# AdmiralenOla/Scoary

Measured on AMD Instinct MI355X. Metric: gene x permutation Fisher tests/sec, higher is better.
Workload: dtype u32 bit-words (bit-sliced adders / AND + popcount), f64 for Fisher p; 1 GPU; cfg3: 50000 genes x 2000 isolates x 10 traits, --permute 10000 per GPU; counts + Fisher + label permutations + exceedance counts; gene_kind=config, gene_order=config, gene_partition=every rank its own genes (weak scaling), genes_per_gpu=50000, genes_total=50000, isolates=2000, traits=10, permutations=10000, parallelism=gene-shard x1, hip_graph=False, hip_graph_auto=False, label_tiles=generated on every rank, exchange=none (single GPU)

## Files before the change

### scoary_amd/csrc/scoary_mfma.hip

```cpp
#include "scoary_common.hpp"

const double kMfmaNsPerGene = 58.0;
const double kListNsPerEntry = 0.18;
const double kMfmaBlockStartStages = 6.0;
const double kMfmaTraitSwitchStages = 2.0;

namespace {

typedef int v8i __attribute__((ext_vector_type(8)));
typedef float v4f __attribute__((ext_vector_type(4)));

constexpr int kBlockGenes = 256;
constexpr int kBlockWaves = 8;
constexpr int kHalfBytes = kStageBytes / 2;
constexpr int kKSteps128 = kKSteps / 2;
constexpr int kKStepBytes = kStageBytes / kKSteps128;
constexpr int kRingSlots = 4;
constexpr int kAhead = kRingSlots - 2;
constexpr int kRingBytes = kRingSlots * kHalfBytes;
constexpr int kDmaPerHalf = kHalfBytes / kBlockWaves / kFragBytes;
constexpr int kThrBytes = 32 * 8;
constexpr int kMfmaLds = kRingBytes + kBlockWaves * kThrBytes;
static_assert(kRingSlots >= 4 && kMfmaLds <= 160 * 1024 && (kAhead - 1) * kDmaPerHalf < 64,
              "a half stage is issued at least two ticks ahead, within the LDS of a CU and the vmcnt field");

__global__ __launch_bounds__(256) void k_mfma_panels(const uint32_t* __restrict__ tiled, int64_t Gp, int G, int N,
                                                     const int32_t* __restrict__ order,
                                                     const uint8_t* __restrict__ flipped, int64_t total,
                                                     v4i* __restrict__ panels) {
  const int64_t idx = (int64_t)blockIdx.x * 256 + threadIdx.x;
  if (idx >= total) return;
  const int lane = (int)(idx & 63);
  const int64_t f = idx >> 6;
  const int k = (int)(f & 31), i = (int)((f >> 5) & 1);
  const int64_t slot = (f >> 6) * 64 + i * 32 + (lane & 31);
  const int w = 2 * k + (lane >> 5);
  uint32_t bits = 0u;
  if (slot < G && 32 * w < N) {
    const int g = order[slot];
    bits = tiled[((int64_t)(w >> 2) * Gp + g) * 4 + (w & 3)];
    if (flipped[g]) bits = ~bits;
    if (32 * w + 32 > N) bits &= (1u << (N - 32 * w)) - 1u;
  }
  panels[idx] = fp4_of_bits32(bits);
}

__global__ __launch_bounds__(256) void k_mfma_bfrag(const uint32_t* __restrict__ tiles, int N, int ntiles,
                                                    int64_t tile_dwords, int S, v4i* __restrict__ bfrag) {
  const int s = blockIdx.x, t = blockIdx.y;
  const int wave = __builtin_amdgcn_readfirstlane(threadIdx.x >> 6);
  const uint32_t* tile = tiles + ((int64_t)t * ntiles + (s >> 3)) * tile_dwords + 2 * (s & 7);
#pragma unroll
  for (int j = 0; j < 2; ++j)
    mfma_bfrag_emit(bfrag, S, t, s, j, wave, 4, [&](int row) { return row < N ? tile[(int64_t)row * 16 + j] : 0u; });
}

__device__ __forceinline__ void mfma_dma16(uint32_t lds, uint32_t lane_off, const unsigned char* src) {
  uint32_t m0_saved;
  asm volatile("s_mov_b32 %0, m0\n\ts_mov_b32 m0, %1\n\ts_nop 0\n\t"
               "global_load_lds_dwordx4 %2, %3\n\ts_mov_b32 m0, %0"
               : "=&s"(m0_saved)
               : "s"(lds), "v"(lane_off), "s"(src)
               : "memory");
}

__device__ __forceinline__ void mfma_dma4(uint32_t lds, uint32_t lane_off, const unsigned char* src) {
  uint32_t m0_saved;
  asm volatile("s_mov_b32 %0, m0\n\ts_mov_b32 m0, %1\n\ts_nop 0\n\t"
               "global_load_lds_dword %2, %3\n\ts_mov_b32 m0, %0"
               : "=&s"(m0_saved)
               : "s"(lds), "v"(lane_off), "s"(src)
               : "memory");
}

__device__ __forceinline__ int xcd_item(int orig, int n) {
  const int q = n >> 3, r = n & 7, x = orig & 7;
  return (x < r ? x * (q + 1) : r * (q + 1) + (x - r) * q) + (orig >> 3);
}

__global__ __launch_bounds__(kBlockWaves * 64) __attribute__((amdgpu_waves_per_eu(2, 2)))
void k_permute_mfma(const v4i* __restrict__ panels, const unsigned char* __restrict__ bfrag,
                    const uint2* __restrict__ lcrit, int G, int64_t P, int S, int64_t Q, int L, int nblk_genes,
                    int ntiles, int64_t gs, uint16_t* __restrict__ partial) {
  extern __shared__ __attribute__((aligned(16))) unsigned char lds[];
  const int item = xcd_item(blockIdx.x, gridDim.x);
  const int gb = item % nblk_genes, rng = item / nblk_genes;
  const int64_t q0 = (int64_t)rng * L;
  const int ns = (int)min((int64_t)L, Q - q0);
  int t = (int)(q0 / S), s = (int)(q0 % S);
  int jt = rng - (int)((int64_t)t * S / L);
  const int tid = threadIdx.x, lane = tid & 63, quad = lane >> 4, l15 = lane & 15;
  const int wave = __builtin_amdgcn_readfirstlane(tid >> 6);
  const bool late = wave >= kBlockWaves / 2;
  const int wslot0 = gb * kBlockGenes + wave * 32;
  const int rows_mine = min(32, G - wslot0) - 4 * quad;
  v4f negc[2];
  float hw[8];
  const uint32_t lds0 = (uint32_t)(uintptr_t)(const __attribute__((address_space(3))) unsigned char*)lds;
  const uint32_t lane_off = (uint32_t)lane * 16u;
  const int thr_slot0 = min(wslot0, G - 1);
  const uint32_t thr_lds = kRingBytes + (uint32_t)wave * kThrBytes;
  auto fetch_thresholds = [&](int tt) {
    uint32_t l = lane_off;
    asm volatile("" : "+v"(l));
    l >>= 4;
    const uint32_t off = (uint32_t)min((int)(l >> 1), G - 1 - thr_slot0) * 8u + (l & 1u) * 4u;
    mfma_dma4(lds0 + thr_lds, off, reinterpret_cast<const unsigned char*>(lcrit + ((int64_t)tt * G + thr_slot0)));
  };
  auto take_thresholds = [&]() {
    int q4 = 4 * quad, mine = rows_mine;
    asm volatile("" : "+v"(q4), "+v"(mine));
    const uint2* thr = reinterpret_cast<const uint2*>(lds + thr_lds) + q4;
#pragma unroll
    for (int r = 0; r < 8; ++r) {
      const int row = 16 * (r >> 2) + (r & 3);
      const uint2 cr = thr[row];
      negc[r >> 2][r & 3] = -0.5f * (float)((int)cr.x + (int)cr.y - 1);
      hw[r] = row < mine ? 0.5f * (float)((int)cr.y - 1 - (int)cr.x) : 1e30f;
    }
    asm volatile("" : "+v"(negc[0]), "+v"(negc[1]));
#pragma unroll
    for (int r = 0; r < 8; ++r) asm volatile("" : "+v"(hw[r]));
  };
  v4i a[2][kKSteps128];
  {
    fetch_thresholds(t);
    const v4i* ap = panels + ((int64_t)gb * kBlockWaves + wave) * (kKSteps * 64) + (quad >> 1) * 64 + (quad & 1) * 32 + l15;
#pragma unroll
    for (int k = 0; k < kKSteps128; ++k)
#pragma unroll
      for (int i = 0; i < 2; ++i) a[i][k] = ap[k * 128 + i * 16];
#pragma unroll
    for (int k = 0; k < kKSteps128; ++k) asm volatile("" : "+v"(a[0][k]), "+v"(a[1][k]));
    asm volatile("s_waitcnt vmcnt(0)" ::: "memory");
    take_thresholds();
  }

  const unsigned char* bsrc = bfrag + q0 * kStageBytes + wave * (kHalfBytes / kBlockWaves);
  const int nh = 2 * ns;
  auto issue_half = [&](int n) {
    const unsigned char* src = bsrc + (int64_t)min(n, nh - 1) * kHalfBytes;
    const uint32_t dst = lds0 + (uint32_t)(n % kRingSlots) * kHalfBytes + (uint32_t)wave * (kHalfBytes / kBlockWaves);
#pragma unroll
    for (int p = 0; p < kDmaPerHalf; ++p) mfma_dma16(dst + p * kFragBytes, lane_off, src + p * kFragBytes);
  };
#pragma unroll
  for (int n = 0; n < kAhead; ++n) issue_half(n);
  int tick = 0;
  auto next_tick = [&]() {
    asm volatile("s_waitcnt vmcnt(%0)" ::"n"((kAhead - 1) * kDmaPerHalf) : "memory");
    __builtin_amdgcn_s_barrier();
    issue_half(tick + kAhead);
    ++tick;
  };

  uint32_t ex[8];
#pragma unroll
  for (int r = 0; r < 8; ++r) ex[r] = 0u;
  const int ragged = (int)(P - (int64_t)(S - 1) * 64);

  v4f acc[2][4];
  auto region_test = [&](int nvalid) {
    if (nvalid < 64) {
#pragma unroll
      for (int j = 0; j < 4; ++j) {
        const bool v = 16 * j + l15 < nvalid;
#pragma unroll
        for (int r = 0; r < 8; ++r) acc[r >> 2][j][r & 3] = v ? acc[r >> 2][j][r & 3] : __builtin_nanf("");
      }
    }
#pragma unroll
    for (int r = 0; r < 8; ++r)
#pragma unroll
      for (int j = 0; j < 4; ++j) ex[r] += (uint32_t)(__builtin_fabsf(acc[r >> 2][j][r & 3]) > hw[r]);
  };
  const int jt0 = jt;
  auto end_segment = [&](int tt) {
    uint16_t* out = partial + ((int64_t)tt * ntiles + jt) * gs + wslot0;
    int rl = l15, q4 = 4 * quad, mine = rows_mine;
    asm volatile("" : "+v"(rl), "+v"(q4), "+v"(mine));
    uint32_t count = 0u;
#pragma unroll
    for (int r = 0; r < 8; ++r) {
      uint32_t v = ex[r];
#pragma unroll
      for (int off = 8; off > 0; off >>= 1) v += __shfl_xor(v, off);
      ex[r] = 0u;
      count = rl == r ? v : count;
    }
    const int row = 16 * (rl >> 2) + (rl & 3);
    if (rl < 8 && row < mine) out[q4 + row] = (uint16_t)count;
    jt = 0;
  };
  if (late) next_tick();
  int rslot = 0;
  for (int st = 0; st < ns; ++st) {
#pragma unroll
    for (int h = 0; h < 2; ++h) {
      next_tick();
      const unsigned char* bbuf = lds + rslot * kHalfBytes + ((quad >> 1) * 128 + (quad & 1) * 32 + l15) * 16;
      rslot = rslot == kRingSlots - 1 ? 0 : rslot + 1;
      constexpr int kBLead = 3, kFrags = 4 * (kKSteps128 / 2);
      v4i bq[kBLead + 1];
      auto read_b = [&](int f) {
        bq[f % (kBLead + 1)] =
            *reinterpret_cast<const v4i*>(bbuf + (f >> 2) * kKStepBytes + ((f >> 1) & 1) * kFragBytes + (f & 1) * 256);
      };
#pragma unroll
      for (int f = 0; f < kBLead; ++f) read_b(f);
      if (h == 0) {
        __builtin_amdgcn_sched_barrier(0);
        if (st > 0) {
          const bool entered = s == 0;
          region_test(entered ? ragged : 64);
          if (entered) {
            end_segment(t - 1);
            take_thresholds();
          }
        }
        if (s == S - 1 && st + 1 < ns) fetch_thresholds(t + 1);
        __builtin_amdgcn_sched_barrier(0);
      }
#pragma unroll
      for (int f = 0; f < kFrags; ++f) {
        const int k = h * (kKSteps128 / 2) + (f >> 2), j = f & 3;
        if (f + kBLead < kFrags) read_b(f + kBLead);
        __builtin_amdgcn_sched_barrier(0);
        const v4i x = bq[f % (kBLead + 1)];
        const v8i bb = v8i{x.x, x.y, x.z, x.w, 0, 0, 0, 0};
#pragma unroll
        for (int i = 0; i < 2; ++i)
          acc[i][j] = __builtin_amdgcn_mfma_scale_f32_16x16x128_f8f6f4(
              v8i{a[i][k].x, a[i][k].y, a[i][k].z, a[i][k].w, 0, 0, 0, 0}, bb, k == 0 ? negc[i] : acc[i][j], 4, 4, 0, 0,
              0, 0);
        __builtin_amdgcn_sched_barrier(0);
      }
    }
    if (++s == S) s = 0, ++t;
  }
  if (!late) next_tick();
  const bool trait_done = s == 0;
  region_test(trait_done ? ragged : 64);
  asm volatile("s_waitcnt vmcnt(0)" ::: "memory");
  end_segment(trait_done ? t - 1 : t);

  {
    int rl = l15, q4 = 4 * quad, mine = rows_mine;
    asm volatile("" : "+v"(rl), "+v"(q4), "+v"(mine));
    const int row = 16 * (rl >> 2) + (rl & 3);
    const bool stores = rl < 8 && row < mine;
    const int t0 = (int)(q0 / S);
    for (int tt = t0; tt < t; ++tt) {
      uint16_t* out = partial + (int64_t)tt * ntiles * gs + wslot0 + q4 + row;
      for (int tile = (tt == t0 ? jt0 : 0) + 1; tile < ntiles; ++tile)
        if (stores) out[(int64_t)tile * gs] = 0;
    }
  }
}

}

struct MfmaRange {
  int64_t L, ranges, switches;
};
static std::vector<MfmaRange> mfma_ranges(int64_t T, int64_t P, int64_t ntiles) {
  std::vector<MfmaRange> out;
  const int64_t S = (P + 63) / 64, Q = T * S;
  for (int64_t L = std::min<int64_t>(Q, 1023); L >= 1; --L) {
    const int64_t ranges = (Q + L - 1) / L;
    if ((Q + ranges - 1) / ranges != L) continue;
    bool ok = true;
    for (int64_t t = 0; t < std::min(T, L) && ok; ++t) ok = ((t + 1) * S - 1) / L - t * S / L + 1 <= ntiles;
    if (!ok) continue;
    MfmaRange c{L, ranges, 0};
    for (int64_t r = 0; r < std::min(ranges, S); ++r)
      c.switches = std::max(c.switches, (std::min(Q, (r + 1) * L) - 1) / S - r * L / S);
    out.push_back(c);
  }
  return out;
}

static MfmaGeom mfma_pick(const std::vector<MfmaRange>& cands, int num_cu, int64_t gene_blocks, int64_t S,
                          int64_t T) {
  MfmaGeom g{};
  g.stages = S;
  g.Q = T * S;
  g.gene_blocks = gene_blocks;
  for (const MfmaRange& c : cands) {
    const int64_t blocks = gene_blocks * c.ranges;
    const double cost = (double)((blocks + num_cu - 1) / num_cu) *
                        ((double)c.L + kMfmaBlockStartStages + (double)c.switches * kMfmaTraitSwitchStages);
    if (g.L == 0 || cost < g.cost) g.cost = cost, g.ranges = c.ranges, g.L = c.L, g.blocks = blocks;
  }
  return g;
}

MfmaGeom scoary_mfma_geom(int num_cu, int64_t k_split, int64_t T, int64_t P, int64_t ntiles) {
  return mfma_pick(mfma_ranges(T, P, ntiles), num_cu, (k_split + kBlockGenes - 1) / kBlockGenes, (P + 63) / 64, T);
}

int scoary_mfma_launch(scoary_handle h, hipStream_t s, const uint32_t* d_tiles, const void* d_panels, void* d_bfrag,
                       const uint32_t* d_lcrit, uint16_t* d_partial, int64_t k_split, int64_t G, int64_t T,
                       int64_t N, int64_t P, int64_t ntiles, int64_t gs, bool bfrag_ready) {
  const MfmaGeom g = scoary_mfma_geom(h->num_cu, k_split, T, P, ntiles);
  if (g.blocks > 0x7fffffffLL || g.stages > 0x7fffffffLL / 64)
    return fail(h, SCOARY_ERR_SIZE, "scoary_permute_hybrid: grid too large");
  if (!h->mfma_lds_optin) {
    HIP_TRY(h, hipFuncSetAttribute(reinterpret_cast<const void*>(&k_permute_mfma),
                                   hipFuncAttributeMaxDynamicSharedMemorySize, 160 * 1024));
    h->mfma_lds_optin = 1;
  }
  if (!bfrag_ready) {
    KernelTimer kt(h, s, "k_mfma_bfrag");
    hipLaunchKernelGGL(k_mfma_bfrag, dim3((unsigned)g.stages, (unsigned)T), dim3(256), 0, s, d_tiles, (int)N,
                       (int)ntiles, list_tile_dwords(N, 16), (int)g.stages, static_cast<v4i*>(d_bfrag));
  }
  {
    KernelTimer kt(h, s, "k_permute_mfma");
    hipLaunchKernelGGL(k_permute_mfma, dim3((unsigned)g.blocks), dim3(kBlockWaves * 64), kMfmaLds, s,
                       static_cast<const v4i*>(d_panels), static_cast<const unsigned char*>(d_bfrag),
                       reinterpret_cast<const uint2*>(d_lcrit), (int)G, P, (int)g.stages, g.Q, (int)g.L,
                       (int)g.gene_blocks, (int)ntiles, gs, d_partial);
  }
  HIP_TRY(h, hipGetLastError());
  return SCOARY_OK;
}

extern "C" {

int64_t scoary_mfma_max_isolates(void) { return kKSteps * 64; }
int64_t scoary_mfma_panels_bytes(int64_t G, int64_t N) {
  if (G < 1 || N < 1 || N > kKSteps * 64) return 0;
  return round_up(G, kBlockGenes) * (2 * kKSteps * 16);
}
int64_t scoary_mfma_bfrag_bytes(int64_t N, int64_t P, int64_t T) {
  if (N < 1 || N > kKSteps * 64 || P < 1 || T < 1) return 0;
  return T * ((P + 63) / 64) * kStageBytes;
}
int64_t scoary_mfma_breakeven_entries(void) { return (int64_t)std::ceil(kMfmaNsPerGene / kListNsPerEntry); }

int scoary_mfma_panels_build(scoary_handle h, const uint32_t* d_tiled, int64_t G, int64_t N, const int32_t* d_order,
                             const uint8_t* d_flipped, void* d_panels, scoary_stream_t stream) {
  if (!h) return SCOARY_ERR_ARG;
  if (!d_tiled || !d_order || !d_flipped || !d_panels || G < 1 || N < 1)
    return fail(h, SCOARY_ERR_ARG, "scoary_mfma_panels_build: bad argument");
  if (N > kKSteps * 64 || G > 0x7fffffffLL - kBlockGenes)
    return fail(h, SCOARY_ERR_SIZE, "scoary_mfma_panels_build: N > 2048 or G >= 2^31");
  DeviceGuard guard(h->device);
  hipStream_t s = static_cast<hipStream_t>(stream);
  const int64_t total = scoary_mfma_panels_bytes(G, N) / 16;
  KernelTimer kt(h, s, "k_mfma_panels");
  hipLaunchKernelGGL(k_mfma_panels, dim3((unsigned)((total + 255) / 256)), dim3(256), 0, s, d_tiled,
                     scoary_tiled_genes(G), (int)G, (int)N, d_order, d_flipped, total, static_cast<v4i*>(d_panels));
  HIP_TRY(h, hipGetLastError());
  return SCOARY_OK;
}

int scoary_mfma_plan(int num_cu, int64_t k_split, int64_t T, int64_t P, int64_t* out) {
  if (num_cu < 1 || k_split < 1 || T < 1 || P < 1 || !out) return SCOARY_ERR_ARG;
  const MfmaGeom g = scoary_mfma_geom(num_cu, k_split, T, P, (P + 511) / 512);
  out[0] = g.gene_blocks, out[1] = g.ranges, out[2] = g.L, out[3] = g.blocks;
  return SCOARY_OK;
}

int scoary_set_mfma_route(scoary_handle h, int mode) {
  if (!h) return SCOARY_ERR_ARG;
  if (mode < SCOARY_MFMA_ROUTE_NONE || mode > SCOARY_MFMA_ROUTE_AUTO)
    return fail(h, SCOARY_ERR_ARG, "scoary_set_mfma_route: mode is 0 (none), 1 (all) or 2 (auto)");
  h->mfma_route = mode;
  return SCOARY_OK;
}

int64_t scoary_mfma_route(scoary_handle h, const int64_t* block_start, int64_t G, int64_t T, int64_t N, int64_t P) {
  if (!h || G < 1 || T < 1 || P < 1 || N < 1 || N > kKSteps * 64 || h->mfma_route == SCOARY_MFMA_ROUTE_NONE)
    return 0;
  if (h->mfma_route == SCOARY_MFMA_ROUTE_ALL) return G;
  if (!block_start) return 0;
  const int64_t nb = G / kBlockGenes, total = block_start[(G + kBlockGenes - 1) / kBlockGenes];
  const double tests = (double)T * (double)P / 1e5;
  const double stage_ns = kMfmaNsPerGene * h->num_cu * kBlockGenes * 64 / 1e5;
  double best = kListNsPerEntry * (double)total * tests;
  int64_t best_nb = 0;
  const std::vector<MfmaRange> cands = mfma_ranges(T, P, (P + 511) / 512);
  for (int64_t b = 1; b <= nb; ++b) {
    const MfmaGeom g = mfma_pick(cands, h->num_cu, b, (P + 63) / 64, T);
    if (g.blocks < h->num_cu) continue;
    const double cost = g.cost * stage_ns + kListNsPerEntry * (double)(total - block_start[b]) * tests;
    if (cost < best) best = cost, best_nb = b;
  }
  return best_nb * kBlockGenes;
}

}
```

Before: 2059 billion tests/s.

## Specialize MFMA loop for late waves to prefetch next half's B fragments across barrier

After: 2153 billion tests/s, median of 6. +4.5%, better.

```diff
diff --git a/scoary_amd/csrc/scoary_mfma.hip b/scoary_amd/csrc/scoary_mfma.hip
--- a/scoary_amd/csrc/scoary_mfma.hip
+++ b/scoary_amd/csrc/scoary_mfma.hip
@@ -146,12 +146,9 @@
   };
 #pragma unroll
   for (int n = 0; n < kAhead; ++n) issue_half(n);
-  int tick = 0;
-  auto next_tick = [&]() {
+  auto barrier = [&]() {
     asm volatile("s_waitcnt vmcnt(%0)" ::"n"((kAhead - 1) * kDmaPerHalf) : "memory");
     __builtin_amdgcn_s_barrier();
-    issue_half(tick + kAhead);
-    ++tick;
   };
 
   uint32_t ex[8];
@@ -192,53 +189,72 @@
     if (rl < 8 && row < mine) out[q4 + row] = (uint16_t)count;
     jt = 0;
   };
-  if (late) next_tick();
-  int rslot = 0;
-  for (int st = 0; st < ns; ++st) {
-#pragma unroll
-    for (int h = 0; h < 2; ++h) {
-      next_tick();
-      const unsigned char* bbuf = lds + rslot * kHalfBytes + ((quad >> 1) * 128 + (quad & 1) * 32 + l15) * 16;
-      rslot = rslot == kRingSlots - 1 ? 0 : rslot + 1;
-      constexpr int kBLead = 3, kFrags = 4 * (kKSteps128 / 2);
-      v4i bq[kBLead + 1];
-      auto read_b = [&](int f) {
-        bq[f % (kBLead + 1)] =
-            *reinterpret_cast<const v4i*>(bbuf + (f >> 2) * kKStepBytes + ((f >> 1) & 1) * kFragBytes + (f & 1) * 256);
-      };
-#pragma unroll
-      for (int f = 0; f < kBLead; ++f) read_b(f);
-      if (h == 0) {
-        __builtin_amdgcn_sched_barrier(0);
-        if (st > 0) {
-          const bool entered = s == 0;
-          region_test(entered ? ragged : 64);
-          if (entered) {
-            end_segment(t - 1);
-            take_thresholds();
+  const unsigned char* lbase = lds + ((quad >> 1) * 128 + (quad & 1) * 32 + l15) * 16;
+  constexpr int kBLead = 3, kFrags = 4 * (kKSteps128 / 2);
+  auto run = [&](auto group) {
+    constexpr bool kLate = decltype(group)::value;
+    v4i bq[kBLead + 1];
+    auto read_b = [&](const unsigned char* buf, int f) {
+      bq[f % (kBLead + 1)] =
+          *reinterpret_cast<const v4i*>(buf + (f >> 2) * kKStepBytes + ((f >> 1) & 1) * kFragBytes + (f & 1) * 256);
+    };
+    int rslot = 0;
+    int nx = kAhead;
+    const unsigned char* bbuf = lbase;
+    if (kLate) {
+      barrier();
+#pragma unroll
+      for (int f = 0; f < kBLead; ++f) read_b(bbuf, f);
+    }
+    for (int st = 0; st < ns; ++st) {
+#pragma unroll
+      for (int h = 0; h < 2; ++h) {
+        if (!kLate) {
+          barrier();
+          issue_half(nx++);
+#pragma unroll
+          for (int f = 0; f < kBLead; ++f) read_b(bbuf, f);
+        }
+        if (h == 0) {
+          __builtin_amdgcn_sched_barrier(0);
+          if (st > 0) {
+            const bool entered = s == 0;
+            region_test(entered ? ragged : 64);
+            if (entered) {
+              end_segment(t - 1);
+              take_thresholds();
+            }
           }
+          if (s == S - 1 && st + 1 < ns) fetch_thresholds(t + 1);
+          __builtin_amdgcn_sched_barrier(0);
         }
-        if (s == S - 1 && st + 1 < ns) fetch_thresholds(t + 1);
-        __builtin_amdgcn_sched_barrier(0);
+        if (kLate) issue_half(nx++);
+        rslot = rslot == kRingSlots - 1 ? 0 : rslot + 1;
+        const unsigned char* nbuf = lbase + rslot * kHalfBytes;
+#pragma unroll
+        for (int f = 0; f < kFrags; ++f) {
+          const int k = h * (kKSteps128 / 2) + (f >> 2), j = f & 3;
+          if (kLate && f == kFrags / 2) barrier();
+          if (f + kBLead < kFrags) read_b(bbuf, f + kBLead);
+          else if (kLate) read_b(nbuf, f + kBLead - kFrags);
+          __builtin_amdgcn_sched_barrier(0);
+          const v4i x = bq[f % (kBLead + 1)];
+          const v8i bb = v8i{x.x, x.y, x.z, x.w, 0, 0, 0, 0};
+#pragma unroll
+          for (int i = 0; i < 2; ++i)
+            acc[i][j] = __builtin_amdgcn_mfma_scale_f32_16x16x128_f8f6f4(
+                v8i{a[i][k].x, a[i][k].y, a[i][k].z, a[i][k].w, 0, 0, 0, 0}, bb, k == 0 ? negc[i] : acc[i][j], 4, 4, 0,
+                0, 0, 0);
+          __builtin_amdgcn_sched_barrier(0);
+        }
+        bbuf = nbuf;
       }
-#pragma unroll
-      for (int f = 0; f < kFrags; ++f) {
-        const int k = h * (kKSteps128 / 2) + (f >> 2), j = f & 3;
-        if (f + kBLead < kFrags) read_b(f + kBLead);
-        __builtin_amdgcn_sched_barrier(0);
-        const v4i x = bq[f % (kBLead + 1)];
-        const v8i bb = v8i{x.x, x.y, x.z, x.w, 0, 0, 0, 0};
-#pragma unroll
-        for (int i = 0; i < 2; ++i)
-          acc[i][j] = __builtin_amdgcn_mfma_scale_f32_16x16x128_f8f6f4(
-              v8i{a[i][k].x, a[i][k].y, a[i][k].z, a[i][k].w, 0, 0, 0, 0}, bb, k == 0 ? negc[i] : acc[i][j], 4, 4, 0, 0,
-              0, 0);
-        __builtin_amdgcn_sched_barrier(0);
-      }
-    }
-    if (++s == S) s = 0, ++t;
-  }
-  if (!late) next_tick();
+      if (++s == S) s = 0, ++t;
+    }
+    if (!kLate) barrier();
+  };
+  if (late) run(std::true_type{});
+  else run(std::false_type{});
   const bool trait_done = s == 0;
   region_test(trait_done ? ragged : 64);
   asm volatile("s_waitcnt vmcnt(0)" ::: "memory");
```
